# mozack/vdjer

Hardware: AMD Instinct MI355X
Metric: M paired-reads/sec (k-mer build + contig score), IgH 50bp PE (higher is better)
Workload: dtype u8/u64 (2-bit packed bases, integer counts)

## Files before the change

vdjer_amd/csrc/vdjx_kmer.hip:

```cpp
#include "vdjx_common.h"
#include "vdjx_scan.h"
#include "vdjx_part.h"

#include <algorithm>
#include <numeric>
#include <type_traits>
#include <string.h>
#include <stdlib.h>

#define HIST_THREADS 512
#define HIST_BLOCKS 512u
#define LOCAL_SLOTS 2048u
#define K3_SUB_TUPLES g_sub_tuples
__device__ u32 g_sub_tuples = 262144u;
#define NONE32 0xFFFFFFFFu
#define INST_MASK 0x7FFFFFFFu

struct RecView {
	u64 bhi, blo, nm, lq;
};

__device__ inline RecView load_rec(const u64* __restrict__ bases, const u64* __restrict__ nmask,
                                   const u64* __restrict__ lowq, size_t r) {
	RecView v;
// ... 47 lines not shown
	return -1;
}

#define INST_BITS 38
#define INST_MASK64 ((1ull << INST_BITS) - 1ull)
#define NONE64 0xFFFFFFFFFFFFFFFFull

struct Tup16 {
	u64 lo, x;
	typedef u32 hi_t;
	__device__ inline u64 hi() const { return x >> INST_BITS; }
	__device__ inline u64 inst() const { return x & INST_MASK64; }
	__device__ static inline Tup16 make(u64 lo, u64 hi, u64 inst) { Tup16 t; t.lo = lo; t.x = (hi << INST_BITS) | inst; return t; }
	__device__ static inline Tup16 load(const Tup16* p) { const ulonglong2 v = *(const ulonglong2*) p; Tup16 t; t.lo = v.x; t.x = v.y; return t; }
	__device__ static inline void store(Tup16* p, const Tup16& t) { *(ulonglong2*) p = make_ulonglong2(t.lo, t.x); }
};
struct Tup24 {
	u64 lo, h, i;
	typedef u64 hi_t;
	__device__ inline u64 hi() const { return h; }
	__device__ inline u64 inst() const { return i; }
	__device__ static inline Tup24 make(u64 lo, u64 hi, u64 inst) { Tup24 t; t.lo = lo; t.h = hi; t.i = inst; return t; }
	__device__ static inline Tup24 load(const Tup24* p) { return *p; }
	__device__ static inline void store(Tup24* p, const Tup24& t) { *p = t; }
};

__device__ inline u64 vdjx_clean_offsets(u64 bad, int k, int P) {
	u64 inv = bad;
	int cur = 1;
	while (cur * 2 <= k) { inv |= inv >> cur; cur *= 2; }
	inv |= inv >> (k - cur);
	return ~inv & (P >= 64 ? ~0ull : (1ull << P) - 1ull);
}

#define GL_WAVE_BYTES 3072u

#define GL_ROW_LONG (VDJX_LONG_W + 2)
#define GL_WAVE_BYTES_LONG (64u * GL_ROW_LONG * 8u + 2048u)
struct GateView { u64 bhi, blo, bad; };
__device__ inline GateView load_gate(const u64* __restrict__ bases, const u64* __restrict__ gate, size_t r) {
	GateView v;
	const ulonglong2 b = ((const ulonglong2*) bases)[r];
	v.bhi = b.x; v.blo = b.y;
	v.bad = gate[r];
	return v;
}
__device__ inline vdjx_mask3 load_gate3(const u64* __restrict__ gate, size_t r) {
	vdjx_mask3 b;
	b.w0 = gate[r * VDJX_LONG_M]; b.w1 = gate[r * VDJX_LONG_M + 1]; b.w2 = gate[r * VDJX_LONG_M + 2];
	return b;
}
__device__ inline vdjx_mask3 load_bad3(const u64* __restrict__ nmask, const u64* __restrict__ lowq, size_t r) {
	vdjx_mask3 b;
	b.w0 = nmask[r * VDJX_LONG_M] | (lowq ? lowq[r * VDJX_LONG_M] : 0ull);
	b.w1 = nmask[r * VDJX_LONG_M + 1] | (lowq ? lowq[r * VDJX_LONG_M + 1] : 0ull);
	b.w2 = nmask[r * VDJX_LONG_M + 2] | (lowq ? lowq[r * VDJX_LONG_M + 2] : 0ull);
	return b;
}
__device__ inline void stage_row_long(u64* row, const u64* __restrict__ bases, size_t r) {
#pragma unroll
	for (int w = 0; w < VDJX_LONG_W; w++) row[w] = bases[r * VDJX_LONG_W + w];
	row[VDJX_LONG_W] = 0; row[VDJX_LONG_W + 1] = 0;
}

__device__ inline bool sym_canonical(const ulonglong2 f, int rl, int k, int o, u64& khi, u64& klo) {
	u64 xh, xl, yh, yl;
	vdjx_kmer_at_lane(f.x, f.y, rl, k, o, xh, xl);
	vdjx_kmer_rc(xh, xl, k, yh, yl);
	const bool flip = yh < xh || (yh == xh && yl < xl);
	khi = flip ? yh : xh;
	klo = flip ? yl : xl;
	return flip;
}

template <bool LONG, bool SYM = false, bool SAMPLED = false>
__global__ __launch_bounds__(HIST_THREADS) void k_gated_hist(const u64* __restrict__ bases, const u64* __restrict__ nmask,
                                                             const u64* __restrict__ lowq, size_t R, int rl, int k, u32 nb_bits,
                                                             size_t rpb, u32* __restrict__ bucket_cnt, u32 dbg_in,
                                                             u32 S, size_t Rv, u32* __restrict__ sampled) {
#ifdef VDJX_ABLATE
	const u32 dbg = dbg_in;
#else
	const u32 dbg = 0u;
#endif
	u32 sink = 0;
	extern __shared__ __attribute__((aligned(16))) u32 hist[];
	const u32 NB = 1u << nb_bits;
	for (u32 i = threadIdx.x; i < NB; i += HIST_THREADS) hist[i] = 0;
	__syncthreads();
	static_assert(!(LONG && SYM), "SYM is the short-read form");
	uint8_t* wv = (uint8_t*) (hist + NB) + (threadIdx.x >> 6) * (LONG ? GL_WAVE_BYTES_LONG : GL_WAVE_BYTES);
	ulonglong2* wb = (ulonglong2*) wv;
	u64* wrow = (u64*) wv;
	uint16_t* wl = (uint16_t*) (wv + (LONG ? 64u * GL_ROW_LONG * 8u : 1024u));
	const u32 lane = threadIdx.x & 63u;
	const size_t r0 = (size_t) blockIdx.x * rpb;
	const size_t r1 = SAMPLED ? (r0 + rpb < Rv ? r0 + rpb : Rv) : (r0 + rpb < R ? r0 + rpb : R);
	const int P = rl - k + 1;
	static_assert(!(LONG && SAMPLED), "the sample is taken of short reads");
	u32 wtot = 0;
	for (size_t rb = r0; rb < r1; rb += HIST_THREADS) {
		const size_t v = rb + threadIdx.x;
		const size_t r = SAMPLED ? ((((v >> 6) * S + S / 2) << 6) | (v & 63)) : v;
		u64 G = 0;
		vdjx_mask3 bad{~0ull, ~0ull, ~0ull};
		if (v < r1 && (!SAMPLED || r < R)) {
			if (LONG) { bad = load_gate3(lowq, r); stage_row_long(wrow + lane * GL_ROW_LONG, bases, r); }
			else {
				const GateView v = load_gate(bases, lowq, SYM ? 2 * r : r);
				G = vdjx_clean_offsets(v.bad, k, P);
				wb[lane] = make_ulonglong2(v.bhi, v.blo);
			}
		}
		constexpr int LSTEP = 16;
		for (int ob = 0; ob < P; ob += LSTEP) {
			const u32 g = LONG ? vdjx_clean16(bad, ob, k, P) : (u32) (G >> ob) & 0xFFFFu;
			const u32 c = (u32) __popc(g);
			const u32 incl = (u32) vdjx_wave_scan_add((int) c);
			const u32 total = (u32) __builtin_amdgcn_readlane((int) incl, 63);
			if (dbg == 1) { sink += incl; continue; }
			if (!total) continue;
			if (SAMPLED) wtot += total;
			u32 at = incl - c;
			for (u32 gg = g; gg; gg &= gg - 1) wl[at++] = (uint16_t) ((lane << (LONG ? 8 : 6)) | (u32) (ob + __builtin_ctz(gg)));
			vdjx_wave_lds_fence();
			if (dbg == 2) { sink += wl[lane]; vdjx_wave_lds_fence(); continue; }
			for (u32 i = lane; i < total; i += 64) {
				const u32 e = wl[i];
				u64 khi, klo;
				if (LONG) vdjx_kmer_at_words(wrow + (e >> 8) * GL_ROW_LONG, k, (int) (e & 255u), khi, klo);
				else if (SYM) (void) sym_canonical(wb[e >> 6], rl, k, (int) (e & 63u), khi, klo);
				else {
					const ulonglong2 bb = wb[e >> 6];
					vdjx_kmer_at_lane(bb.x, bb.y, rl, k, (int) (e & 63u), khi, klo);
				}
				if (dbg == 3) { sink += (u32) (vdjx_bucket_mix(klo, khi) >> (64 - nb_bits)); continue; }
				atomicAdd(&hist[(u32) (vdjx_bucket_mix(klo, khi) >> (64 - nb_bits))], 1u);
			}
			vdjx_wave_lds_fence();
		}
	}
	__syncthreads();
	if (dbg) { if (sink == 0x12345u) bucket_cnt[0] = sink; return; }
	for (u32 i = threadIdx.x; i < NB; i += HIST_THREADS) if (hist[i]) atomicAdd(&bucket_cnt[i], hist[i]);
	if (SAMPLED && lane == 0 && wtot) atomicAdd(sampled, wtot);
}

template <typename TUP> struct TupBucket {
	u32 shift, mask;
	__device__ inline u32 operator()(const TUP& t) const { return (u32) (vdjx_bucket_mix(t.lo, t.hi()) >> shift) & mask; }
};

#define PARTR_STAGE_BYTES 98304u
template <typename TUP, bool LONG, bool SYM = false>
__global__ __launch_bounds__(PART_THREADS) void k_part_records_g(const u64* __restrict__ bases, const u64* __restrict__ nmask,
                                                                 const u64* __restrict__ lowq, size_t R, u64 rec_base, int rl, int k,
                                                                 u32 shift, u32 nbk, size_t rpb, u32 rr0, const u32* __restrict__ lim, u32 lsh,
                                                                 u32* __restrict__ over, u32* __restrict__ gcur, TUP* __restrict__ out) {
	extern __shared__ __attribute__((aligned(16))) uint8_t smem[];
	TUP* stage = (TUP*) smem;
	u32* desc = (u32*) (smem + PARTR_STAGE_BYTES);
	__shared__ part_round pr;
	__shared__ u32 s_n;
	constexpr u32 ROUND = PARTR_STAGE_BYTES / sizeof(TUP);
	constexpr int OB = LONG ? 8 : 6;
	const int P = rl - k + 1;
	const u32 rr_min = ROUND / (u32) P;
	u32 rr = rr0 > rr_min ? rr0 : rr_min;
	const u32 mask = nbk - 1;
	const u32 lane = threadIdx.x & 63u, wave = threadIdx.x >> 6;
	static_assert(!(LONG && SYM), "SYM is the short-read form");
	uint8_t* wv = smem + wave * (LONG ? GL_WAVE_BYTES_LONG : GL_WAVE_BYTES);
	ulonglong2* wb = (ulonglong2*) wv;
	u64* wrow = (u64*) wv;
	uint16_t* wl = (uint16_t*) (wv + (LONG ? 64u * GL_ROW_LONG * 8u : 1024u));
	const size_t r0 = (size_t) blockIdx.x * rpb;
	const size_t r1 = r0 + rpb < R ? r0 + rpb : R;
	size_t rs = r0;
	pr.limits(nbk, lim, lsh, over);
	while (rs < r1) {
		const size_t re = rs + rr < r1 ? rs + rr : r1;
		if (threadIdx.x == 0) s_n = 0;
		pr.begin(nbk);
		for (size_t rb = rs; rb < re; rb += PART_THREADS) {
			const size_t r = rb + threadIdx.x;
			u64 G = 0;
			vdjx_mask3 bad{~0ull, ~0ull, ~0ull};
			if (r < re) {
				if (LONG) { bad = load_gate3(lowq, r); stage_row_long(wrow + lane * GL_ROW_LONG, bases, r); }
				else {
					const GateView v = load_gate(bases, lowq, SYM ? 2 * r : r);
					G = vdjx_clean_offsets(v.bad, k, P);
					wb[lane] = make_ulonglong2(v.bhi, v.blo);
				}
			}
			const u32 loc0 = (u32) (rb - rs) + wave * 64u;
			constexpr int LSTEP = 16;
			for (int ob = 0; ob < P; ob += LSTEP) {
				const u32 g = LONG ? vdjx_clean16(bad, ob, k, P) : (u32) (G >> ob) & 0xFFFFu;
				const u32 c = (u32) __popc(g);
				const u32 incl = (u32) vdjx_wave_scan_add((int) c);
				const u32 total = (u32) __builtin_amdgcn_readlane((int) incl, 63);
				if (!total) continue;
				u32 at = incl - c;
				for (u32 gg = g; gg; gg &= gg - 1) wl[at++] = (uint16_t) ((lane << OB) | (u32) (ob + __builtin_ctz(gg)));
				vdjx_wave_lds_fence();
				u32 dbase = 0;
				if (lane == 0) dbase = atomicAdd(&s_n, total);
				dbase = (u32) __builtin_amdgcn_readlane((int) dbase, 0);
				for (u32 i = lane; i < total; i += 64) {
					const u32 e = wl[i];
					u64 khi, klo;
					if (LONG) vdjx_kmer_at_words(wrow + (e >> 8) * GL_ROW_LONG, k, (int) (e & 255u), khi, klo);
					else if (SYM) (void) sym_canonical(wb[e >> 6], rl, k, (int) (e & 63u), khi, klo);
					else {
						const ulonglong2 bb = wb[e >> 6];
						vdjx_kmer_at_lane(bb.x, bb.y, rl, k, (int) (e & 63u), khi, klo);
					}
					const u32 b = (u32) (vdjx_bucket_mix(klo, khi) >> shift) & mask;
					pr.count(b);
					if (dbase + i < ROUND) desc[dbase + i] = ((loc0 + (e >> OB)) << (OB + 10)) | ((e & ((1u << OB) - 1u)) << 10) | b;
				}
				vdjx_wave_lds_fence();
			}
		}
		__syncthreads();
		if (s_n > ROUND) {
			rr = rr / 2 > rr_min ? rr / 2 : rr_min;
			__syncthreads();
			continue;
		}
		const u32 n = pr.reserve(nbk, gcur);
		if (n == PART_DEAD) return;
		for (u32 i = threadIdx.x; i < n; i += PART_THREADS) {
			const u32 d = desc[i];
			const size_t r = rs + (d >> (OB + 10));
			const u32 o = (d >> 10) & ((1u << OB) - 1u);
			u64 khi, klo;
			u64 inst = ((rec_base + (u64) r) << OB) | (u64) o;
			if (LONG) vdjx_kmer_at_words(bases + r * VDJX_LONG_W, k, (int) o, khi, klo);
			else if (SYM) {
				const bool flip = sym_canonical(((const ulonglong2*) bases)[2 * r], rl, k, (int) o, khi, klo);
				inst = flip ? ((rec_base + 2 * (u64) r + 1) << OB) | (u64) (rl - k - (int) o) : ((rec_base + 2 * (u64) r) << OB) | (u64) o;
			} else {
				const ulonglong2 bb = ((const ulonglong2*) bases)[r];
				vdjx_kmer_at_lane(bb.x, bb.y, rl, k, (int) o, khi, klo);
			}
			TUP::store(&stage[pr.slot(d & 1023u)], TUP::make(klo, khi, inst));
		}
		__syncthreads();
		pr.flush(stage, n, out, TupBucket<TUP>{shift, mask});
		rs = re;
	}
}

template <typename TUP>
__global__ __launch_bounds__(512) void k_seg_hist_g(const TUP* __restrict__ in, const u32* __restrict__ seg_start, u32 seg_shift, u32 slices,
                                                    u32 shift, u32 sub_bits, u32* __restrict__ fine_cnt, const u32* __restrict__ seg_end,
                                                    const u32* __restrict__ over) {
	__shared__ u32 h[PART_MAXB];
	if (over && *over) return;
	const u32 nbk = 1u << sub_bits;
	for (u32 i = threadIdx.x; i < nbk; i += 512) h[i] = 0;
	__syncthreads();
	size_t t0, t1;
	const u32 seg = part_slice(seg_start, seg_shift, slices, t0, t1, seg_end);
	for (size_t t = t0 + threadIdx.x; t < t1; t += 512) {
		const TUP x = TUP::load(&in[t]);
		atomicAdd(&h[(u32) (vdjx_bucket_mix(x.lo, x.hi()) >> shift) & (nbk - 1)], 1u);
	}
	__syncthreads();
	for (u32 i = threadIdx.x; i < nbk; i += 512) if (h[i]) atomicAdd(&fine_cnt[((size_t) seg << sub_bits) | i], h[i]);
}

#ifndef RD_THREADS
#define RD_THREADS 768
#define RD_UNR 4
#define RD_WAVES 6
#endif
#define RD_SLOTS 2048u
#define RD_SLOT_BITS 11
#define RD_PQ 4096u
#define RD_LI 512u
#define RD_LROWS 128u
#define RD_MAXLOW 11u
#define ST_CAND 1u
#define ST_MULTI 2u
#define ST_QOK 4u
#define ST_QOK_R 8u
#define ST_ID_SHIFT 8
#define ST_NOID 0xFFFFFFu

struct SurvOutG { u64* lo; u64* hi; u32* gcnt; u64* gfirst; u32* n; u32 cap; u32* n_real; };
#define GC_SHADOW 0x80000000u
#define GC_MASK 0x7FFFFFFFu

__device__ inline bool reads_equal(const u64* __restrict__ bases, const u64* __restrict__ nmask, int rl, u64 a, u64 b) {
	if (rl <= VDJX_SHORT_READ_LEN) {
		const ulonglong2 x = ((const ulonglong2*) bases)[a];
		const ulonglong2 y = ((const ulonglong2*) bases)[b];
		return x.x == y.x && x.y == y.y && nmask[a] == nmask[b];
	}
	u64 d = 0;
#pragma unroll
	for (int w = 0; w < VDJX_LONG_W; w++) d |= bases[a * VDJX_LONG_W + w] ^ bases[b * VDJX_LONG_W + w];
#pragma unroll
	for (int w = 0; w < VDJX_LONG_M; w++) d |= nmask[a * VDJX_LONG_M + w] ^ nmask[b * VDJX_LONG_M + w];
	return d == 0;
}

__device__ inline u32 rd_hash(u64 lo, u64 hi) {
	u32 x = (u32) lo ^ ((u32) (lo >> 32) * 0x9E3779B1u) ^ (((u32) hi ^ (u32) (hi >> 32) * 0x27D4EB2Fu) * 0x85EBCA6Bu);
	x ^= x >> 15; x *= 0xC2B2AE35u; x ^= x >> 13;
	return x;
}

__device__ inline u32 rd_count_min(u32* cnt, u64* mn, u32 idx, u64 val, bool active) {
	u32 c0 = 0;
	const u64 act = __ballot(active);
	if (act) {
		const int leader = __ffsll((long long) act) - 1;
		const u32 lidx = (u32) __builtin_amdgcn_readlane((int) idx, leader);
		const bool same = active && idx == lidx;
		const u64 m = __ballot(same);
		if (__popcll(m) >= 8) {
			const u32 hi_min = vdjx_wave_min(same ? (u32) (val >> 32) : 0xFFFFFFFFu);
			const u32 lo_min = vdjx_wave_min(same && (u32) (val >> 32) == hi_min ? (u32) val : 0xFFFFFFFFu);
			u32 old = 0;
			if (__lane_id() == leader) {
				old = atomicAdd(&cnt[lidx], (u32) __popcll(m));
				atomicMin((unsigned long long*) &mn[lidx], ((unsigned long long) hi_min << 32) | lo_min);
			}
			old = (u32) __builtin_amdgcn_readlane((int) old, leader);
			if (same) c0 = old + (u32) __popcll(m & ((1ull << __lane_id()) - 1ull));
			active = active && !same;
		}
	}
	if (active) { c0 = atomicAdd(&cnt[idx], 1u); atomicMin((unsigned long long*) &mn[idx], (unsigned long long) val); }
	return c0;
}

__global__ __launch_bounds__(1024) void k_bucket_order(const u32* __restrict__ bucket_start, const u32* __restrict__ bucket_end, u32 NB, u32* __restrict__ order) {
	__shared__ u32 cls_cnt[33], cls_at[33];
	if (threadIdx.x < 33) cls_cnt[threadIdx.x] = 0;
	__syncthreads();
	for (u32 b = threadIdx.x; b < NB; b += 1024) {
		const u32 n = bucket_end[b] - bucket_start[b];
		atomicAdd(&cls_cnt[n ? 32u - (u32) __builtin_clz(n) : 0u], 1u);
	}
	__syncthreads();
	if (threadIdx.x == 0) { u32 at = 0; for (int cl = 32; cl >= 0; cl--) { cls_at[cl] = at; at += cls_cnt[cl]; } }
	__syncthreads();
	for (u32 b = threadIdx.x; b < NB; b += 1024) {
		const u32 n = bucket_end[b] - bucket_start[b];
		order[atomicAdd(&cls_at[n ? 32u - (u32) __builtin_clz(n) : 0u], 1u)] = b;
	}
}

template <typename TUP, bool SYM = false>
__global__ __launch_bounds__(RD_THREADS, sizeof(TUP) == 16 ? RD_WAVES : RD_WAVES / 2) void k_gated_reduce(const TUP* __restrict__ tup, const u32* __restrict__ bucket_start,
                                                             const u32* __restrict__ bucket_end, const u32* __restrict__ cut_over,
                                                             const u64* __restrict__ bases, const u64* __restrict__ nmask,
                                                             vdjx_qrows quals, int rl, int ob, int k, u64 rec_base,
                                                             u32 mf, u32 cmin, u32 mqq, u32 tlow, SurvOutG so,
                                                             u64* __restrict__ g_distinct, u32* __restrict__ g_err, u32 dbg_in,
                                                             const u32* __restrict__ order) {
#ifdef VDJX_ABLATE
	const u32 dbg = dbg_in;
#else
	const u32 dbg = dbg_in == 9u ? 9u : 0u;
#endif
	typedef typename TUP::hi_t THI;
	__shared__ u64 s_klo[RD_SLOTS];
	__shared__ THI s_khi[RD_SLOTS];
	__shared__ u64 s_first[RD_SLOTS];
	__shared__ u32 s_cnt[RD_SLOTS], s_state[RD_SLOTS];
	__shared__ u32 pq[RD_PQ];
	__shared__ u64 low_inst[RD_LI];
	__shared__ u32 low_n[RD_LROWS];
	__shared__ unsigned short low_slot[RD_LROWS];
	__shared__ u32 s_over, s_ndist, s_nlow, s_npq, s_nsurv, s_base, s_nreal;
	const THI EMPTY = (THI) ~(THI) 0;
	if (cut_over && *cut_over) return;
	const u32 b = order ? order[blockIdx.x] : blockIdx.x;
	const u32 base = bucket_start[b];
	const u32 n = bucket_end[b] - base;
	const u32 tid = threadIdx.x;
	if (n == 0) return;
	const TUP* T = tup + base;
	const u32 om = (1u << ob) - 1u;
	const u32 per_low = tlow > 1 ? (tlow - 1 < RD_MAXLOW ? tlow - 1 : RD_MAXLOW) : 1;
	const u32 lrows = RD_LI / per_low < RD_LROWS ? RD_LI / per_low : RD_LROWS;
	u32 S = 1;
	while ((u64) S * K3_SUB_TUPLES < n) S <<= 1;
	u32 ndist_total = 0;
	bool verify = S > 1;
	for (;;) {
		if (tid == 0) { s_over = 0; s_ndist = 0; }
		__syncthreads();
		for (u32 s = 0; s < S; s++) {
			for (u32 i = tid; i < RD_SLOTS; i += RD_THREADS) { s_khi[i] = EMPTY; s_cnt[i] = 0; s_first[i] = NONE64; s_state[i] = 0; }
			if (tid == 0) { s_nlow = 0; s_npq = (n >> (32 - RD_SLOT_BITS) || dbg == 9) ? RD_PQ + 1 : 0; s_nsurv = 0; s_nreal = 0; }
			__syncthreads();
			for (u32 t0 = 0; t0 < n; t0 += RD_UNR * RD_THREADS) {
// ... 1519 lines not shown
#define CUT_MARGIN_FLOOR 264u
#define CUT_SAMPLE_MIN_RECORDS ((size_t) 1 << 20)
struct cut_cap {
	u32 S, floor;
	float cS;
	__device__ u32 operator()(u32 h) const { return S * h + (u32) ceilf(cS * sqrtf((float) h + 1.0f)) + floor; }
};
static float cut_margin_c() { static const float v = CUT_MARGIN_C * (float) vdjx_env_num("VDJX_CUT_MARGIN", 100, 0, 100000) / 100.0f; return v; }
static u32 cut_sample_stride(const vdjx_pool* pool, size_t R) {
	static const bool given = vdjx_env_set("VDJX_HIST_SAMPLE");
	static const u32 S = (u32) vdjx_env_num("VDJX_HIST_SAMPLE", 16, 1, 4096);
	if (pool->W != 2 || S < 2) return 1;
	if (!given && R < CUT_SAMPLE_MIN_RECORDS) return 1;
	return (R + 63) / 64 > S / 2 ? S : 1;
}

template <typename A>
int stage_gated_hist(vdjx_ctx* c, A& db, const vdjx_pool* pool, int k, size_t per_bucket, u64 geometry_instances, GatedHist* gh, bool sym = false, u32 S = 1) {
	hipStream_t st = c->stream;
	const size_t R = sym ? pool->n_records / 2 : pool->n_records;
	const int P = pool->rl - k + 1;
	const u64 NI = geometry_instances ? geometry_instances : (u64) R * (u64) P;
	const size_t per = per_bucket ? per_bucket : gated_bucket_default();
	const u32 hb_max = pool->W > 2 ? 14u : 15u;
	u32 HB = ceil_log2_u64((NI + per - 1) / per);
	HB = std::max(8u, std::min(hb_max, HB));
	const u32 NBH = 1u << HB;
#ifdef VDJX_ABLATE
	static const u32 hist_dbg = (u32) vdjx_env_num("VDJX_HIST_DBG", 0, 0, 4);
#else
	constexpr u32 hist_dbg = 0;
#endif
	const bool lng = pool->W > 2;
	if (lng || per_bucket || geometry_instances || (R + 63) / 64 <= S / 2) S = 1;
	if (S > 1) {
		const double s_max = (double) NI / S + 64.0 * P, cS = (double) cut_margin_c() * S;
		if ((double) S * s_max + (double) NBH * (CUT_MARGIN_FLOOR + 1.0) + cS * sqrt((double) NBH * (s_max + NBH)) >= 4.0e9) S = 1;
	}
	const size_t rows = (R + 63) / 64;
	const size_t Rv = S > 1 ? (rows - S / 2 + S - 1) / S * 64 : R;
	u32 nblk = S > 1 ? (u32) std::min<size_t>(HIST_BLOCKS, (Rv + 1023) / 1024) : (u32) std::min<size_t>(HIST_BLOCKS, (R + 4095) / 4096);
	if (nblk == 0) nblk = 1;
	size_t rpb = (Rv + nblk - 1) / nblk;
	if (S > 1) rpb = (rpb + 63) / 64 * 64;
	u32 *hcnt, *hstart, *blk;
	HIP_TRY(db.alloc(&blk, 2 * (size_t) NBH + 2));
	hstart = blk;
	u32* samp = blk + NBH + 1;
	hcnt = samp + 1;
	HIP_TRY(hipMemsetAsync(samp, 0, ((size_t) NBH + 1) * 4, st));
	const size_t lds_hist = (size_t) NBH * 4 + (HIST_THREADS / 64) * (lng ? GL_WAVE_BYTES_LONG : GL_WAVE_BYTES);
	HIP_TRY(hipFuncSetAttribute((const void*) k_gated_hist<false>, hipFuncAttributeMaxDynamicSharedMemorySize, (int) lds_hist));
	HIP_TRY(hipFuncSetAttribute((const void*) k_gated_hist<true>, hipFuncAttributeMaxDynamicSharedMemorySize, (int) lds_hist));
	HIP_TRY(hipFuncSetAttribute((const void*) k_gated_hist<false, true>, hipFuncAttributeMaxDynamicSharedMemorySize, (int) lds_hist));
	HIP_TRY(hipFuncSetAttribute((const void*) k_gated_hist<false, false, true>, hipFuncAttributeMaxDynamicSharedMemorySize, (int) lds_hist));
	HIP_TRY(hipFuncSetAttribute((const void*) k_gated_hist<false, true, true>, hipFuncAttributeMaxDynamicSharedMemorySize, (int) lds_hist));
	const auto launch_hist = [&](u32 nb, size_t per_blk, u32* cnt, u32 stride, size_t rv, u32* sampled) {
		auto* hist = lng ? k_gated_hist<true> : stride > 1 ? (sym ? k_gated_hist<false, true, true> : k_gated_hist<false, false, true>) : sym ? k_gated_hist<false, true> : k_gated_hist<false>;
		hipLaunchKernelGGL(hist, dim3(nb), dim3(HIST_THREADS), lds_hist, st, pool->d_bases, pool->d_nmask, pool->d_lowq, R, pool->rl, k, HB, per_blk, cnt, hist_dbg, stride, rv, sampled);
	};
	{
		vdjx_prof_scope ps(c, "k_gated_hist");
		launch_hist(nblk, rpb, hcnt, S, Rv, samp);
	}
	dbg_sync(c, "k_gated_hist");
	const cut_cap cap{S, CUT_MARGIN_FLOOR, cut_margin_c() * (float) S};
	if (S > 1 && sync_debug()) {
		u32* exact;
		HIP_TRY(db.alloc(&exact, NBH));
		HIP_TRY(hipMemsetAsync(exact, 0, (size_t) NBH * 4, st));
		const u32 nbe = (u32) std::max<size_t>(1, std::min<size_t>(HIST_BLOCKS, (R + 4095) / 4096));
		launch_hist(nbe, (R + nbe - 1) / nbe, exact, 1u, R, samp);
		std::vector<u32> he(NBH), hs(NBH);
		HIP_TRY(hipMemcpyAsync(he.data(), exact, (size_t) NBH * 4, hipMemcpyDeviceToHost, st));
		HIP_TRY(hipMemcpyAsync(hs.data(), hcnt, (size_t) NBH * 4, hipMemcpyDeviceToHost, st));
		HIP_TRY(hipStreamSynchronize(st));
		double worst = 0, n = 0, caps = 0;
		u32 unseen = 0;
		for (u32 b = 0; b < NBH; b++) {
			worst = std::max(worst, ((double) he[b] - (double) S * hs[b]) / ((double) S * sqrt((double) hs[b] + 1.0)));
			if (!hs[b]) unseen = std::max(unseen, he[b]);
			n += he[b];
			caps += (double) S * hs[b] + ceil((double) cap.cS * sqrt((double) hs[b] + 1.0)) + cap.floor;
		}
		fprintf(stderr, "[vdjx] sampled cut: S %u, 2^%u buckets, %.0f tuples, worst ratio %.3f, largest unseen bucket %u, capacities / tuples %.3f\n", S, HB, n, worst, unseen, n ? caps / n : 0.0);
	}
	if (S > 1) vdjx_scan_one(st, hcnt, NBH, hstart, cap);
	else vdjx_scan_one(st, hcnt, NBH, hstart);
	HIP_TRY(hipMemcpyAsync(c->h_pin, hstart + NBH, 8, hipMemcpyDeviceToHost, st));
	HIP_TRY(hipStreamSynchronize(st));
	HIP_TRY(hipGetLastError());
#ifdef VDJX_ABLATE
	if (hist_dbg) return VDJX_ESTATE;
#endif
	gh->HB = HB; gh->NBH = NBH; gh->hstart = hstart; gh->sym = sym; gh->S = S;
	if (S > 1) {
		const u64 s = ((const u32*) c->h_pin)[1], n_est = (u64) S * s;
		gh->N = (u32) n_est;
		gh->cap_total = *(const u32*) c->h_pin;
		return VDJX_OK;
	}
	const u32 N = *(const u32*) c->h_pin;
	c->stats["gated_instances"] = sym ? 2ull * N : N;
	gh->N = N;
	return VDJX_OK;
}

__global__ __launch_bounds__(1024) void k_cut_totals(const u32* __restrict__ bucket_start, const u32* __restrict__ bucket_end, u32 NB,
                                                     const u32* __restrict__ over, u32* __restrict__ over_out, unsigned long long* __restrict__ total) {
	__shared__ u32 wsum[16];
	const u32 b = blockIdx.x * 1024u + threadIdx.x;
	const u32 n = b < NB ? bucket_end[b] - bucket_start[b] : 0u;
	const u32 incl = (u32) vdjx_wave_scan_add((int) n);
	if ((threadIdx.x & 63u) == 63u) wsum[threadIdx.x >> 6] = incl;
	__syncthreads();
	if (threadIdx.x == 0) {
		unsigned long long t = 0;
		for (u32 w = 0; w < 16; w++) t += wsum[w];
		if (t) atomicAdd(total, t);
		if (blockIdx.x == 0) *over_out = *over;
	}
}

template <typename TUP, typename A>
int stage_gated_cut(vdjx_ctx* c, A& db, const vdjx_pool* pool, u64 rec_base, int k, size_t per_bucket, u64 geometry_instances, const GatedHist& gh, GTuples<TUP>* out) {
	hipStream_t st = c->stream;
	const bool sym = gh.sym;
	const size_t R = sym ? pool->n_records / 2 : pool->n_records;
	const int P = pool->rl - k + 1;
	const size_t per = per_bucket ? per_bucket : gated_bucket_default();
	const u32 hb_max = pool->W > 2 ? 14u : 15u;
	const bool lng = pool->W > 2;
	const u32 HB = gh.HB, NBH = gh.NBH, N = gh.N;
	const bool smp = gh.S > 1;
	const size_t room = smp ? gh.cap_total : N;
	u32* hstart = gh.hstart;
	size_t rpb;
	out->N = (u32) room;
	out->S = gh.S;
	out->Nsurv = smp ? (u32) std::min<u64>(room, (u64) N + (u64) ceil((double) cut_margin_c() * gh.S * sqrt((double) (N / gh.S) + 1.0)) + CUT_MARGIN_FLOOR) : N;
	const u64 Ng = geometry_instances ? geometry_instances : (u64) N;
	static const size_t refine = (size_t) vdjx_env_num("VDJX_REFINE_TUPLES", 4096, 1, 1ll << 32);
	u32 T = 8;
	while (T < HB && ((u64) per << T) < Ng) T++;
	u32 extra = 0;
	const size_t refine_at = per_bucket ? std::max<size_t>(per_bucket, refine / 2) : refine;
	if (T == HB && HB == hb_max && Ng / NBH > refine_at) {
		extra = 1;
		while (extra < 5 && (Ng >> extra) / NBH > refine_at) extra++;
	}
	const u32 Tt = T + extra;
	const u32 NBt = 1u << Tt;
	HIP_TRY(db.alloc(&out->t, room + 1));
	constexpr u32 stage_tuples = PARTR_STAGE_BYTES / (u32) sizeof(TUP);
	constexpr u32 lds_partr = PARTR_STAGE_BYTES + stage_tuples * 4;
	u32 cbits = Tt, fbits = 0;
	if (Tt > 10) { cbits = extra ? Tt - 10 : 8; fbits = Tt - cbits; }
	const u32 NBc = 1u << cbits;
	u32 nblk2 = (u32) std::min<size_t>(1024, (R + 2047) / 2048);
	if (nblk2 == 0) nblk2 = 1;
	rpb = (R + nblk2 - 1) / nblk2;
	u32 *gcur, *over = nullptr;
	HIP_TRY(db.alloc(&gcur, NBc));
	if (smp) {
		HIP_TRY(db.alloc(&over, 1));
		HIP_TRY(hipMemsetAsync(over, 0, 4, st));
	}
	out->over = over;
	TUP* l1 = out->t;
	if (fbits) HIP_TRY(db.alloc(&l1, room + 1));
	{
		vdjx_prof_scope ps(c, "k_part_records");
		const u64 NIl = (u64) R * (u64) P;
		u64 rr = N ? (u64) stage_tuples * 3 / 4 * NIl / ((u64) N * (u64) P) : 1u << 16;
		rr = std::max<u64>(PART_THREADS, std::min<u64>(rr / PART_THREADS * PART_THREADS, lng ? 1u << 14 : 1u << 16));
		auto* part_records = lng ? k_part_records_g<TUP, true> : sym ? k_part_records_g<TUP, false, true> : k_part_records_g<TUP, false>;
		HIP_TRY(part_launch(st, part_records, nblk2, lds_partr, hstart, NBc, HB - cbits, gcur, l1, pool->d_bases, pool->d_nmask, pool->d_lowq, R, rec_base,
		                    pool->rl, k, 64 - cbits, NBc, rpb, (u32) rr, smp ? (const u32*) hstart : (const u32*) nullptr, HB - cbits, over));
	}
	dbg_sync(c, "k_part_records");
	u32* tstart;
	HIP_TRY(db.alloc(&tstart, NBt + 1));
	out->NB = NBt;
	out->bucket_start = tstart;
	out->bucket_end = tstart + 1;
	const u32* seg_end = smp ? gcur : nullptr;
	constexpr u32 slices = PART_SLICES;
	if (extra) {
		u32* fine_cnt;
		HIP_TRY(db.alloc(&fine_cnt, NBt));
		HIP_TRY(hipMemsetAsync(fine_cnt, 0, (size_t) NBt * 4, st));
		vdjx_prof_scope ps(c, "k_seg_hist");
		hipLaunchKernelGGL(k_seg_hist_g<TUP>, dim3(NBc * slices), dim3(512), 0, st, l1, hstart, HB - cbits, slices, 64 - Tt, fbits, fine_cnt, seg_end, (const u32*) over);
		vdjx_scan_one(st, fine_cnt, NBt, tstart);
	} else {
		hipLaunchKernelGGL(k_pick_u32, dim3((NBt + 1 + 255) / 256), dim3(256), 0, st, hstart, 1u << (HB - Tt), NBt + 1, tstart);
		if (smp && !fbits) out->bucket_end = gcur;
	}
	if (fbits) {
		u32* gcur2;
		HIP_TRY(db.alloc(&gcur2, NBt));
		const bool lim2 = smp && !extra;
		if (lim2) out->bucket_end = gcur2;
		vdjx_prof_scope ps(c, "k_part_tuples");
		HIP_TRY(part_launch(st, k_part<TUP, TupBucket<TUP>, part_segs>, NBc * slices, PART_LDS_BYTES, tstart, NBt, 0u, gcur2, out->t,
		                    l1, part_segs{hstart, HB - cbits, slices, fbits, seg_end, lim2 ? (const u32*) tstart : (const u32*) nullptr, over}, TupBucket<TUP>{64 - Tt, (1u << fbits) - 1u}));
	}
	return VDJX_OK;
}

template <typename TUP, typename A>
int stage_gated_partition(vdjx_ctx* c, A& db, const vdjx_pool* pool, u64 rec_base, int k, size_t per_bucket, u64 geometry_instances, GTuples<TUP>* out, bool sym = false, u32 S = 1) {
	GatedHist gh;
	int rc = stage_gated_hist(c, db, pool, k, per_bucket, geometry_instances, &gh, sym, S);
	if (rc) return rc;
	return stage_gated_cut<TUP>(c, db, pool, rec_base, k, per_bucket, geometry_instances, gh, out);
}

static int set_sub_tuples(vdjx_ctx* c) {
	static const u32 sub = (u32) vdjx_env_num("VDJX_SUB_TUPLES", 262144, 1, 0xFFFFFFFFll);
	if (c->sub_tuples_set != sub) {
		HIP_TRY(hipMemcpyToSymbolAsync(HIP_SYMBOL(g_sub_tuples), &sub, 4, 0, hipMemcpyHostToDevice, c->stream));
		c->sub_tuples_set = sub;
	}
	return VDJX_OK;
}
template <typename TUP, typename A>
int bucket_order(vdjx_ctx* c, A& db, const GTuples<TUP>& t, u32** order) {
	*order = nullptr;
	if (t.NB < 1024) return VDJX_OK;
	HIP_TRY(db.alloc(order, t.NB));
	hipLaunchKernelGGL(k_bucket_order, dim3(1), dim3(1024), 0, c->stream, t.bucket_start, t.bucket_end, t.NB, *order);
	return VDJX_OK;
}

template <typename TUP, typename A>
int stage_gated_reduce(vdjx_ctx* c, A& db, GTuples<TUP>& t, const PoolView& pv, u64 rec_base, int k, int mf, int mq, SurvivorsG* sv, bool sym = false) {
	hipStream_t st = c->stream;
	int rc = set_sub_tuples(c);
	if (rc) return rc;
	if (mq >= 255) mq = 254;
	const u32 mqq = (u32) (mq < 0 ? 0 : (mq > 214 ? 214 : mq));
	const u32 tlow = 1 + (mqq + 19) / 20;
	const u32 cmin = (u32) std::max(mf, 2);
	const u32 mfu = (u32) std::max(mf, 0);
	const u32 cap = (sym ? t.Nsurv : t.Nsurv / 2) + 16;
	u32 *g_err, *n_surv;
	u64* g_distinct;
	HIP_TRY(db.alloc(&sv->lo, cap)); HIP_TRY(db.alloc(&sv->hi, cap)); HIP_TRY(db.alloc(&sv->gcnt, cap)); HIP_TRY(db.alloc(&sv->gfirst, cap));
	HIP_TRY(db.alloc(&g_distinct, 64 * 16 + 3));
	g_err = (u32*) (g_distinct + 64 * 16);
	n_surv = g_err + 1;
	u32* n_real = g_err + 2;
	HIP_TRY(hipMemsetAsync(g_distinct, 0, (64 * 16 + 3) * 8, st));
	if (t.over) hipLaunchKernelGGL(k_cut_totals, dim3((t.NB + 1023) / 1024), dim3(1024), 0, st, t.bucket_start, t.bucket_end, t.NB, (const u32*) t.over, g_err + 3,
	                               (unsigned long long*) (g_distinct + 64 * 16 + 2));
	SurvOutG so{sv->lo, sv->hi, sv->gcnt, sv->gfirst, n_surv, cap, n_real};
	static const u32 rd_dbg = (u32) vdjx_env_num("VDJX_RD_DBG", 0, 0, 9);
	if (t.N) {
		vdjx_prof_scope ps(c, "k_gated_reduce");
		u32* order;
		if ((rc = bucket_order(c, db, t, &order))) return rc;
		if (sym) hipLaunchKernelGGL((k_gated_reduce<TUP, true>), dim3(t.NB), dim3(RD_THREADS), 0, st, t.t, t.bucket_start, t.bucket_end, (const u32*) t.over, pv.bases, pv.nmask, pv.quals, pv.rl, pv.ob, k, rec_base,
		                            mfu, cmin, mqq, tlow, so, g_distinct, g_err, rd_dbg, (const u32*) order);
		else hipLaunchKernelGGL(k_gated_reduce<TUP>, dim3(t.NB), dim3(RD_THREADS), 0, st, t.t, t.bucket_start, t.bucket_end, (const u32*) t.over, pv.bases, pv.nmask, pv.quals, pv.rl, pv.ob, k, rec_base,
		                        mfu, cmin, mqq, tlow, so, g_distinct, g_err, rd_dbg, (const u32*) order);
	}
	u64* spread = (u64*) c->h_pin;
	u32* tail = (u32*) (spread + 64 * 16);
	static_assert((64 * 16 + 3) * 8 == VDJX_HPIN_SYNC_BYTES, "h_pin layout (vdjx_common.h)");
	HIP_TRY(hipMemcpyAsync(spread, g_distinct, VDJX_HPIN_SYNC_BYTES, hipMemcpyDeviceToHost, st));
	HIP_TRY(hipStreamSynchronize(st));
	HIP_TRY(hipGetLastError());
	const u32 ns = tail[1], err = tail[0];
	if (t.over) {
		if (tail[3] || ns > cap) return VDJX_ECUT;
		t.N = (u32) spread[64 * 16 + 2];
		c->stats["gated_instances"] = sym ? 2ull * t.N : t.N;
	}
	if (err) { vdjx_set_error("k_gated_reduce: %u buckets could not be split to fit LDS", err); return VDJX_EHIP; }
	if (ns > cap) { vdjx_set_error("survivor capacity logic failed (%u > %u)", ns, cap); return VDJX_EHIP; }
	sv->ndist = 0;
	for (int i = 0; i < 64; i++) sv->ndist += spread[i * 16];
	sv->n = ns;
	sv->n_real = sym ? tail[2] : ns;
	c->stats["kmer_build_shadows"] = ns - sv->n_real;
	return VDJX_OK;
}

struct RecountOut { u32* ucnt; u64* ufirst; u64* in_first; u32* in_from; u64* edge_first; u32* edge_to; };
struct RecountStatus { const u32* g_err = nullptr; const u32* n_items = nullptr; const unsigned long long* n_inst = nullptr; u32 ns = 0; };
#define VDJX_ESYMWALK (-1000)
static int recount_status_check(vdjx_ctx* c, const u32* hp, u32 ns) {
	if (hp[6] || hp[7]) { vdjx_set_error("the mirrored walk found %u + %u places where the chains are not mirror images", hp[6], hp[7]); return VDJX_ESYMWALK; }
	if (hp[0]) { vdjx_set_error("k_walk_items: item buffer too small (%u waves stopped)", hp[0]); return VDJX_EHIP; }
	if (hp[1]) { vdjx_set_error("internal error: %u of %u surviving k-mers were not met again in the records (VDJX_SYNC_DEBUG=1 names them)", hp[1], ns); return VDJX_EHIP; }
	c->stats["recount_items"] = hp[2];
	c->stats["recount_instances"] = *(const unsigned long long*) (hp + 4);
	return VDJX_OK;
}

template <typename A>
int stage_recount(vdjx_ctx* c, A& db, const vdjx_pool* pool, u64 rec_base, int k, SurvivorsG& sv, const RecountOut& ro,
                  bool derive_edges, SurvTable* table_out = nullptr, RecountStatus* defer = nullptr, bool sym_walk = false) {
	hipStream_t st = c->stream;
	const size_t R = pool->n_records;
	const int P = pool->rl - k + 1;
	const u32 ns = sv.n;
	if (ns >= (1u << 26)) { vdjx_set_error("more than 2^26 surviving k-mers: not supported by the recount items"); return VDJX_ELIMIT; }
	if (R >= (1ull << 29)) { vdjx_set_error("more than 2^29 records on one GPU: not supported by the recount items"); return VDJX_ELIMIT; }
	if ((u64) R * (u64) P >= (1ull << 32)) { vdjx_set_error("records*offsets = %llu >= 2^32 on one GPU: shard the pool over more GPUs", (unsigned long long) ((u64) R * (u64) P)); return VDJX_ELIMIT; }
	u32 tmask = 1023;
	while ((size_t) tmask + 1 < (size_t) ns * 2) tmask = tmask * 2 + 1;
	unsigned long long* pred;
	ulonglong2* table;
	u32 *succ0, *succ, *bloom, *clen, *coff, *newidx, *jump_open, *fbw, *gcnt2, *bestsucc, *partner = nullptr;
	u64 *pd, *lo2, *hi2, *gfirst2, *linw;
	ulonglong2 *skey0, *skey;
	u32 bloom_bits = 1u << 16;
	while (bloom_bits < (1u << 30) && (size_t) bloom_bits < (size_t) ns * 16) bloom_bits <<= 1;
	const u32 nb16 = (ns + 15u) >> 4;
	const u32 n_jump = (ceil_log2_u64((u64) ns + 1) + 4) / 5 + 1;
	{
		auto up = [](size_t b) { return (b + 255) & ~(size_t) 255; };
		const size_t b_bloom = up(bloom_bits / 8), b_table = up(((size_t) tmask + 1) * 16), b_pred = up((size_t) ns * 8), b_clen = up((size_t) ns * 4),
		             b_jump = up((size_t) (n_jump + 1) * 4), b_linw = up(((size_t) nb16 + 1) * 8);
		uint8_t* z;
		const size_t zb = b_bloom + b_table + b_pred + b_clen + b_jump + b_linw;
// ... 1084 lines not shown
```

vdjer_amd/csrc/vdjx_part.h:

```cpp
#pragma once

#include "vdjx_common.h"

#include <type_traits>

#define PART_THREADS 1024
#define PART_LDS_BYTES 131072
#define PART_MAXB 1024
#define PART_SLICES 8u
#define PART_NONE 0xFFFFFFFFu
#define PART_HOLE 0xFFFFFFFFFFFFFFFFull
#define PART_DEAD 0xFFFFFFFFu

namespace {

__device__ inline void part_scan(const u32* cnt, u32* base, u32* tmp, u32 n) {
	const u32 t = threadIdx.x, lane = t & 63, wv = t >> 6;
	const u32 a = 2 * t < n ? cnt[2 * t] : 0, b = 2 * t + 1 < n ? cnt[2 * t + 1] : 0;
	const u32 incl = (u32) vdjx_wave_scan_add((int) (a + b));
	if (lane == 63) tmp[wv] = incl;
	__syncthreads();
	if (wv == 0) {
		const u32 w = lane < PART_THREADS / 64 ? tmp[lane] : 0;
		const u32 wi = (u32) vdjx_wave_scan_add((int) w);
		if (lane < PART_THREADS / 64) tmp[lane] = wi - w;
		if (lane == 63) tmp[PART_THREADS / 64] = wi;
	}
	__syncthreads();
	const u32 excl = tmp[wv] + incl - (a + b);
	if (2 * t < n) base[2 * t] = excl;
	if (2 * t + 1 < n) base[2 * t + 1] = excl + a;
	if (t == 0) base[n] = tmp[PART_THREADS / 64];
	__syncthreads();
}

template <typename T> __device__ inline T part_load(const T* p) { return T::load(p); }
template <typename T> __device__ inline void part_store(T* p, const T& x) { T::store(p, x); }
__device__ inline u64 part_load(const u64* p) { return *p; }
__device__ inline void part_store(u64* p, const u64& x) { *p = x; }

struct part_round {
	u32 cnt[PART_MAXB], base[PART_MAXB + 1], cur[PART_MAXB], gbase[PART_MAXB], tmp[PART_THREADS];
	u32 end[PART_MAXB];
	u32* over;
	u32 dead, stop;

	__device__ inline bool limits(u32 nbk, const u32* __restrict__ lim, u32 lsh, u32* word, const u32* seen = nullptr) {
		if (lim) for (u32 i = threadIdx.x; i < nbk; i += PART_THREADS) end[i] = lim[((size_t) i + 1) << lsh];
		if (threadIdx.x == 0) {
			over = lim ? word : nullptr;
			stop = seen ? __hip_atomic_load(seen, __ATOMIC_RELAXED, __HIP_MEMORY_SCOPE_AGENT) : 0u;
		}
		__syncthreads();
		return stop != 0;
	}

	__device__ inline void begin(u32 nbk) {
		for (u32 i = threadIdx.x; i < nbk; i += PART_THREADS) cnt[i] = 0;
		if (threadIdx.x == 0) dead = 0;
		__syncthreads();
	}
	__device__ inline void count(u32 b) { atomicAdd(&cnt[b], 1u); }
	__device__ inline u32 reserve(u32 nbk, u32* __restrict__ gcur) {
		part_scan(cnt, base, tmp, nbk);
		u32* const word = over;
		for (u32 i = threadIdx.x; i < nbk; i += PART_THREADS) {
			cur[i] = base[i];
			const u32 n = cnt[i];
			const u32 g = n ? atomicAdd(&gcur[i], n) : 0u;
			gbase[i] = g;
			if (word && (u64) g + n > (u64) end[i]) { dead = 1; atomicExch(word, 1u); }
		}
		__syncthreads();
		return dead ? PART_DEAD : base[nbk];
	}
	__device__ inline u32 slot(u32 b) { return atomicAdd(&cur[b], 1u); }
	template <typename T, typename Key> __device__ inline void flush(const T* stage, u32 n, T* __restrict__ out, const Key& key) {
		for (u32 i = threadIdx.x; i < n; i += PART_THREADS) {
			const T x = part_load(&stage[i]);
			const u32 b = key(x);
			part_store(&out[gbase[b] + (i - base[b])], x);
		}
		__syncthreads();
	}
};

__device__ inline u32 part_slice(const u32* __restrict__ seg_start, u32 seg_shift, u32 slices, size_t& t0, size_t& t1, const u32* __restrict__ seg_end = nullptr) {
	const u32 seg = blockIdx.x / slices, sl = blockIdx.x % slices;
	const size_t s0 = seg_start[(size_t) seg << seg_shift], s1 = seg_end ? seg_end[seg] : seg_start[((size_t) seg + 1) << seg_shift];
	const size_t per = (s1 - s0 + slices - 1) / slices;
	t0 = s0 + (size_t) sl * per;
	t1 = t0 + per < s1 ? t0 + per : s1;
	return seg;
}

struct part_share {
	const unsigned long long* n;
	u32 nbk;
	__device__ inline size_t span(u32 round, size_t& t0, size_t& t1, u32& buckets) const {
		const size_t N = (size_t) *n;
		const size_t per = ((N + gridDim.x - 1) / gridDim.x + round - 1) / round * round;
		t0 = (size_t) blockIdx.x * per;
		t1 = t0 + per < N ? t0 + per : N;
		buckets = nbk;
		return 0;
	}
	__device__ inline const u32* limits(size_t) const { return nullptr; }
	__device__ inline u32* over_word() const { return nullptr; }
};
struct part_segs {
	const u32* seg_start;
	u32 seg_shift, slices, sub_bits;
	const u32* seg_end = nullptr;
	const u32* lim = nullptr;
	u32* over = nullptr;
	__device__ inline size_t span(u32, size_t& t0, size_t& t1, u32& buckets) const {
		buckets = 1u << sub_bits;
		return (size_t) part_slice(seg_start, seg_shift, slices, t0, t1, seg_end) << sub_bits;
	}
	__device__ inline const u32* limits(size_t first) const { return lim ? lim + first : nullptr; }
	__device__ inline u32* over_word() const { return over; }
};

template <typename T, typename Key, typename Range, bool PAIRED = false>
__global__ __launch_bounds__(PART_THREADS) void k_part(const T* __restrict__ in, Range range, Key key, u32* __restrict__ gcur, T* __restrict__ out) {
	extern __shared__ __attribute__((aligned(16))) uint8_t part_smem[];
	T* stage = (T*) part_smem;
	__shared__ part_round pr;
	constexpr u32 PER = PART_LDS_BYTES / sizeof(T) / PART_THREADS;
	constexpr u32 ROUND = PER * PART_THREADS;
	static_assert(!PAIRED || (std::is_same<T, u64>::value && PER % 2 == 0), "the paired loads are for 8-byte elements");
	size_t t0, t1;
	u32 nbk;
	const size_t first = range.span(ROUND, t0, t1, nbk);
	u32* gc = gcur + first;
	if (pr.limits(nbk, range.limits(first), 0u, range.over_word(), range.over_word())) return;
	for (size_t ts = t0; ts < t1; ts += ROUND) {
		const size_t te = ts + ROUND < t1 ? ts + ROUND : t1;
		pr.begin(nbk);
		T r_x[PER];
		u32 r_b[PER];
		if constexpr (PAIRED) {
#pragma unroll
			for (u32 j = 0; j < PER; j += 2) {
				const size_t t = ts + ((size_t) (j / 2) * PART_THREADS + threadIdx.x) * 2;
				r_x[j] = PART_HOLE; r_x[j + 1] = PART_HOLE;
				if (t + 1 < te) { const ulonglong2 v = *(const ulonglong2*) &in[t]; r_x[j] = v.x; r_x[j + 1] = v.y; }
				else if (t < te) r_x[j] = in[t];
			}
#pragma unroll
			for (u32 j = 0; j < PER; j++) {
				r_b[j] = PART_NONE;
				if (r_x[j] != PART_HOLE) { r_b[j] = key(r_x[j]); pr.count(r_b[j]); }
			}
		} else {
#pragma unroll
			for (u32 j = 0; j < PER; j++) {
				const size_t t = ts + (size_t) j * PART_THREADS + threadIdx.x;
				r_b[j] = PART_NONE;
				if (t < te) { r_x[j] = part_load(&in[t]); r_b[j] = key(r_x[j]); }
			}
#pragma unroll
			for (u32 j = 0; j < PER; j++) if (r_b[j] != PART_NONE) pr.count(r_b[j]);
		}
		__syncthreads();
		const u32 n = pr.reserve(nbk, gc);
		if (n == PART_DEAD) return;
#pragma unroll
		for (u32 j = 0; j < PER; j++) if (r_b[j] != PART_NONE) part_store(&stage[pr.slot(r_b[j])], r_x[j]);
		__syncthreads();
		pr.flush(stage, n, out, key);
	}
}

__global__ void k_init_cursors(const u32* __restrict__ bucket_start, u32 n, u32 sh, u32* __restrict__ cur) {
	u32 i = blockIdx.x * blockDim.x + threadIdx.x;
	if (i < n) cur[i] = bucket_start[(size_t) i << sh];
}

template <typename... P, typename O, typename... Args>
inline hipError_t part_launch(hipStream_t st, void (*kernel)(P...), u32 grid, u32 lds, const u32* bucket_start, u32 ncur, u32 sh, u32* gcur, O* out,
                              Args... args) {
	const hipError_t e = hipFuncSetAttribute((const void*) kernel, hipFuncAttributeMaxDynamicSharedMemorySize, (int) lds);
	if (e != hipSuccess) return e;
	hipLaunchKernelGGL(k_init_cursors, dim3((ncur + 255) / 256), dim3(256), 0, st, bucket_start, ncur, sh, gcur);
	hipLaunchKernelGGL(kernel, dim3(grid), dim3(PART_THREADS), lds, st, args..., gcur, out);
	return hipSuccess;
}

}
```

Before: 944.9.

## Keep short-read k-mer tuples in LDS instead of recomputing them for the scatter

For short reads, the partition kernel now builds each k-mer tuple once in the first pass and stores it in LDS along with a 16-bit bucket id. The second pass no longer re-reads bases from global memory and recomputes k-mers. It instead sorts indices by bucket slot and copies the stored tuples to their output positions. This removes a global reload and the repeated k-mer extraction, at the cost of a smaller round size (more LDS per tuple) and an indirect gather from LDS. The part_round scratch array is also shrunk, and the host-side round sizing is adjusted to match.

```diff
diff --git a/profiles/kcalls.py b/profiles/kcalls.py
--- /dev/null
+++ b/profiles/kcalls.py
@@ -0,0 +1,16 @@
+#!/usr/bin/env python3
+import csv
+import glob
+import sys
+
+d = sys.argv[1]
+want = sys.argv[2:] or ["k_gated_hist", "k_part_records_g", "k_seg_hist_g", "k_part<", "k_gated_reduce"]
+rows = [r for f in glob.glob(d + "/**/*kernel_trace.csv", recursive=True) for r in csv.DictReader(open(f))]
+by = {}
+for r in rows:
+    name = r["Kernel_Name"].replace("(anonymous namespace)::", "")
+    if any(w in name for w in want):
+        by.setdefault(name.split("(")[0], []).append((int(r["End_Timestamp"]) - int(r["Start_Timestamp"])) / 1e3)
+for name, v in sorted(by.items()):
+    print(f"{name} | {len(v)} calls, mean {sum(v) / len(v):.1f}, {min(v):.1f}-{max(v):.1f} us")
+print(f"all kernels of the process: {sum(int(r['End_Timestamp']) - int(r['Start_Timestamp']) for r in rows) / 1e6:.3f} ms in {len(rows)} dispatches")
diff --git a/vdjer_amd/csrc/vdjx_kmer.hip b/vdjer_amd/csrc/vdjx_kmer.hip
--- a/vdjer_amd/csrc/vdjx_kmer.hip
+++ b/vdjer_amd/csrc/vdjx_kmer.hip
@@ -223,17 +223,25 @@
 };
 
 #define PARTR_STAGE_BYTES 98304u
+#define PARTR_LIST_BYTES (PART_THREADS / 64u * GL_WAVE_BYTES)
+#define PARTR_KEEP_BYTES 93600u
+template <typename TUP, bool LONG> constexpr u32 partr_round() { return LONG ? PARTR_STAGE_BYTES / (u32) sizeof(TUP) : PARTR_KEEP_BYTES / ((u32) sizeof(TUP) + 2u); }
+template <typename TUP, bool LONG> constexpr u32 partr_lds() { return LONG ? PARTR_STAGE_BYTES + partr_round<TUP, true>() * 4u : PARTR_LIST_BYTES + PARTR_KEEP_BYTES; }
 template <typename TUP, bool LONG, bool SYM = false>
 __global__ __launch_bounds__(PART_THREADS) void k_part_records_g(const u64* __restrict__ bases, const u64* __restrict__ nmask,
                                                                  const u64* __restrict__ lowq, size_t R, u64 rec_base, int rl, int k,
                                                                  u32 shift, u32 nbk, size_t rpb, u32 rr0, const u32* __restrict__ lim, u32 lsh,
                                                                  u32* __restrict__ over, u32* __restrict__ gcur, TUP* __restrict__ out) {
 	extern __shared__ __attribute__((aligned(16))) uint8_t smem[];
-	TUP* stage = (TUP*) smem;
-	u32* desc = (u32*) (smem + PARTR_STAGE_BYTES);
+	constexpr bool KEEP = !LONG;
+	constexpr u32 ROUND = partr_round<TUP, LONG>();
+	static_assert(PARTR_LIST_BYTES % 16 == 0 && ROUND * sizeof(TUP) % 8 == 0 && ROUND * 4u <= PARTR_LIST_BYTES && ROUND <= 65536u, "the KEEP layout");
+	static_assert(PART_THREADS / 64u * GL_WAVE_BYTES_LONG <= PARTR_STAGE_BYTES, "the long lists live in the stage");
+	TUP* stage = (TUP*) (smem + (KEEP ? PARTR_LIST_BYTES : 0u));
+	u32* desc = (u32*) (smem + (KEEP ? 0u : PARTR_STAGE_BYTES));
+	uint16_t* bkt = (uint16_t*) (stage + ROUND);
 	__shared__ part_round pr;
 	__shared__ u32 s_n;
-	constexpr u32 ROUND = PARTR_STAGE_BYTES / sizeof(TUP);
 	constexpr int OB = LONG ? 8 : 6;
 	const int P = rl - k + 1;
 	const u32 rr_min = ROUND / (u32) P;
@@ -281,16 +289,27 @@
 				dbase = (u32) __builtin_amdgcn_readlane((int) dbase, 0);
 				for (u32 i = lane; i < total; i += 64) {
 					const u32 e = wl[i];
+					const u32 o = e & ((1u << OB) - 1u);
 					u64 khi, klo;
-					if (LONG) vdjx_kmer_at_words(wrow + (e >> 8) * GL_ROW_LONG, k, (int) (e & 255u), khi, klo);
-					else if (SYM) (void) sym_canonical(wb[e >> 6], rl, k, (int) (e & 63u), khi, klo);
-					else {
-						const ulonglong2 bb = wb[e >> 6];
-						vdjx_kmer_at_lane(bb.x, bb.y, rl, k, (int) (e & 63u), khi, klo);
+					if constexpr (LONG) {
+						vdjx_kmer_at_words(wrow + (e >> 8) * GL_ROW_LONG, k, (int) o, khi, klo);
+						const u32 b = (u32) (vdjx_bucket_mix(klo, khi) >> shift) & mask;
+						pr.count(b);
+						if (dbase + i < ROUND) desc[dbase + i] = ((loc0 + (e >> OB)) << (OB + 10)) | (o << 10) | b;
+					} else {
+						const u64 r = rec_base + (SYM ? 2 : 1) * (u64) (rs + loc0 + (e >> OB));
+						u64 inst = (r << OB) | (u64) o;
+						const ulonglong2 bb = wb[e >> OB];
+						if (SYM) {
+							if (sym_canonical(bb, rl, k, (int) o, khi, klo)) inst = ((r + 1) << OB) | (u64) (rl - k - (int) o);
+						} else vdjx_kmer_at_lane(bb.x, bb.y, rl, k, (int) o, khi, klo);
+						const u32 b = (u32) (vdjx_bucket_mix(klo, khi) >> shift) & mask;
+						pr.count(b);
+						if (dbase + i < ROUND) {
+							TUP::store(&stage[dbase + i], TUP::make(klo, khi, inst));
+							bkt[dbase + i] = (uint16_t) b;
+						}
 					}
-					const u32 b = (u32) (vdjx_bucket_mix(klo, khi) >> shift) & mask;
-					pr.count(b);
-					if (dbase + i < ROUND) desc[dbase + i] = ((loc0 + (e >> OB)) << (OB + 10)) | ((e & ((1u << OB) - 1u)) << 10) | b;
 				}
 				vdjx_wave_lds_fence();
 			}
@@ -303,24 +322,30 @@
 		}
 		const u32 n = pr.reserve(nbk, gcur);
 		if (n == PART_DEAD) return;
-		for (u32 i = threadIdx.x; i < n; i += PART_THREADS) {
-			const u32 d = desc[i];
-			const size_t r = rs + (d >> (OB + 10));
-			const u32 o = (d >> 10) & ((1u << OB) - 1u);
-			u64 khi, klo;
-			u64 inst = ((rec_base + (u64) r) << OB) | (u64) o;
-			if (LONG) vdjx_kmer_at_words(bases + r * VDJX_LONG_W, k, (int) o, khi, klo);
-			else if (SYM) {
-				const bool flip = sym_canonical(((const ulonglong2*) bases)[2 * r], rl, k, (int) o, khi, klo);
-				inst = flip ? ((rec_base + 2 * (u64) r + 1) << OB) | (u64) (rl - k - (int) o) : ((rec_base + 2 * (u64) r) << OB) | (u64) o;
-			} else {
-				const ulonglong2 bb = ((const ulonglong2*) bases)[r];
-				vdjx_kmer_at_lane(bb.x, bb.y, rl, k, (int) o, khi, klo);
-			}
-			TUP::store(&stage[pr.slot(d & 1023u)], TUP::make(klo, khi, inst));
+		if constexpr (LONG) {
+			for (u32 i = threadIdx.x; i < n; i += PART_THREADS) {
+				const u32 d = desc[i];
+				const size_t r = rs + (d >> (OB + 10));
+				const u32 o = (d >> 10) & ((1u << OB) - 1u);
+				u64 khi, klo;
+				vdjx_kmer_at_words(bases + r * VDJX_LONG_W, k, (int) o, khi, klo);
+				TUP::store(&stage[pr.slot(d & 1023u)], TUP::make(klo, khi, ((rec_base + (u64) r) << OB) | (u64) o));
+			}
+			__syncthreads();
+			pr.flush(stage, n, out, TupBucket<TUP>{shift, mask});
+		} else {
+			u32* sorted = desc;
+			for (u32 i = threadIdx.x; i < n; i += PART_THREADS) {
+				const u32 b = bkt[i];
+				sorted[pr.slot(b)] = (b << 16) | i;
+			}
+			__syncthreads();
+			for (u32 j = threadIdx.x; j < n; j += PART_THREADS) {
+				const u32 s = sorted[j], b = s >> 16;
+				TUP::store(&out[pr.gbase[b] + (j - pr.base[b])], TUP::load(&stage[s & 0xFFFFu]));
+			}
+			__syncthreads();
 		}
-		__syncthreads();
-		pr.flush(stage, n, out, TupBucket<TUP>{shift, mask});
 		rs = re;
 	}
 }
@@ -2146,8 +2171,6 @@
 	const u32 Tt = T + extra;
 	const u32 NBt = 1u << Tt;
 	HIP_TRY(db.alloc(&out->t, room + 1));
-	constexpr u32 stage_tuples = PARTR_STAGE_BYTES / (u32) sizeof(TUP);
-	constexpr u32 lds_partr = PARTR_STAGE_BYTES + stage_tuples * 4;
 	u32 cbits = Tt, fbits = 0;
 	if (Tt > 10) { cbits = extra ? Tt - 10 : 8; fbits = Tt - cbits; }
 	const u32 NBc = 1u << cbits;
@@ -2165,9 +2188,12 @@
 	if (fbits) HIP_TRY(db.alloc(&l1, room + 1));
 	{
 		vdjx_prof_scope ps(c, "k_part_records");
+		const u32 round_tuples = lng ? partr_round<TUP, true>() : partr_round<TUP, false>();
+		const u32 lds_partr = lng ? partr_lds<TUP, true>() : partr_lds<TUP, false>();
 		const u64 NIl = (u64) R * (u64) P;
-		u64 rr = N ? (u64) stage_tuples * 3 / 4 * NIl / ((u64) N * (u64) P) : 1u << 16;
-		rr = std::max<u64>(PART_THREADS, std::min<u64>(rr / PART_THREADS * PART_THREADS, lng ? 1u << 14 : 1u << 16));
+		u64 rr = N ? (lng ? (u64) round_tuples * 3 / 4 : (u64) round_tuples * 7 / 8) * NIl / ((u64) N * (u64) P) : 1u << 16;
+		const u64 rstep = lng ? PART_THREADS : 64u;
+		rr = std::max<u64>(rstep, std::min<u64>(rr / rstep * rstep, lng ? 1u << 14 : 1u << 16));
 		auto* part_records = lng ? k_part_records_g<TUP, true> : sym ? k_part_records_g<TUP, false, true> : k_part_records_g<TUP, false>;
 		HIP_TRY(part_launch(st, part_records, nblk2, lds_partr, hstart, NBc, HB - cbits, gcur, l1, pool->d_bases, pool->d_nmask, pool->d_lowq, R, rec_base,
 		                    pool->rl, k, 64 - cbits, NBc, rpb, (u32) rr, smp ? (const u32*) hstart : (const u32*) nullptr, HB - cbits, over));
diff --git a/vdjer_amd/csrc/vdjx_part.h b/vdjer_amd/csrc/vdjx_part.h
--- a/vdjer_amd/csrc/vdjx_part.h
+++ b/vdjer_amd/csrc/vdjx_part.h
@@ -40,7 +40,8 @@
 __device__ inline void part_store(u64* p, const u64& x) { *p = x; }
 
 struct part_round {
-	u32 cnt[PART_MAXB], base[PART_MAXB + 1], cur[PART_MAXB], gbase[PART_MAXB], tmp[PART_THREADS];
+	u32 cnt[PART_MAXB], base[PART_MAXB + 1], cur[PART_MAXB], gbase[PART_MAXB];
+	u32 tmp[PART_THREADS / 64 + 1];
 	u32 end[PART_MAXB];
 	u32* over;
 	u32 dead, stop;
```

After: 960.5, median of 6. 1.6% higher.
